# ShioMisaka/fce-yolo

Hardware: AMD Instinct MI355X
Metric: images/sec/GPU @ 640x640 bs=32, yolo11n-fce; fraction of fp16 MFMA roofline (higher is better)
Workload: dtype fp16; 1 GPU; yolo11n-fce detection inference (forward + decode + NMS) @ 640x640, 32 images/GPU; model=yolo11n-fce, global_batch=32, imgsz=640, parallelism=dp1, batches_in_flight=4, distinct_inputs=5, hw_queues=8, forward_launch=hipgraph

## Files before the change

fce-yolo_amd/_native.py:

```python

from __future__ import annotations

import ctypes as C
import os
from pathlib import Path

LIB_PATH = Path(__file__).resolve().parent / "lib" / "libfceyolo.so"

F16, F32, U8 = 0, 1, 2
NHWC, NCHW = 0, 1
ACT_NONE, ACT_SILU = 0, 1
EPI_STORE, EPI_WSTORE, EPI_ACCUM = 0, 1, 2
PLAN_NO_AUTOTUNE = 1


class FceError(RuntimeError):
    pass


class Tensor(C.Structure):
    _fields_ = [
        ("data", C.c_void_p),
        ("dtype", C.c_int),
        ("layout", C.c_int),
# ... 100 lines not shown
        ("w", C.c_void_p * 2),
        ("b", C.c_void_p * 2),
        ("epi1", C.c_int),
        ("fw", C.c_void_p),
        ("fn", C.c_int),
        ("fi", C.c_int),
    ]


class NmsOpts(C.Structure):
    _fields_ = [
        ("conf_thres", C.c_float),
        ("iou_thres", C.c_float),
        ("max_det", C.c_int),
        ("max_nms", C.c_int),
        ("max_wh", C.c_float),
        ("agnostic", C.c_int),
        ("multi_label", C.c_int),
        ("classes", C.c_void_p),
        ("nclasses", C.c_int),
    ]


_P = C.c_void_p
_I = C.c_int
_SZ = C.c_size_t
_PT = C.POINTER(Tensor)
_PCD = C.POINTER(ConvDesc)
_PCO = C.POINTER(CoordDesc)
_PC3 = C.POINTER(C3k2Desc)
_PDC = C.POINTER(DclsDesc)
_PST = C.POINTER(Stem2Desc)
_PBN = C.POINTER(BneckDesc)
_PPW = C.POINTER(Pw2Desc)

_SIGS = {
    "fce_last_error": (C.c_char_p, []),
    "fce_abi_version": (_I, []),
    "fce_device_count": (_I, []),
    "fce_conv_weight_bytes": (_SZ, [_PCD]),
    "fce_conv_pack_weights": (_I, [_PCD, _P, _P]),
    "fce_conv2d": (_I, [_PCD, _PT, _P, _P, _PT, _PT, _P]),
    "fce_conv_variants": (_I, [_PCD, _I, _P, _I]),
    "fce_letterbox": (_I, [_P, _I, _P, _I, _I, _I, _P]),
    "fce_scale_boxes": (_I, [_P, _P, _I, _I, _P, _P]),
    "fce_conv2d_variant": (_I, [_PCD, _PT, _P, _P, _PT, _PT, _I, _P]),
    "fce_conv2d_variant_dup": (_I, [_PCD, _PT, _P, _P, _PT, _PT, _I, _PT, _I, _P]),
    "fce_conv2d_detect": (_I, [_PCD, _PT, _P, _P, C.POINTER(DetectEpi), _P]),
    "fce_maxpool_chain": (_I, [_PT, _PT, _PT, _PT, _I, _P]),
    "fce_weighted_add": (_I, [_PT, _I, _P, _I, _I, _I, _PT, _P]),
    "fce_coord_workspace_bytes": (_SZ, [_PCO, _I, _I, _I]),
    "fce_c3k2_supported": (_I, [_PC3]),
    "fce_c3k2": (_I, [_PC3, _PT, _PT, _P]),
    "fce_net_add_c3k2": (_I, [_P, _PC3, _I, _I, _I, _I]),
    "fce_net_add_c3k2_alt": (_I, [_P, _PC3, _I, _I, _I, _I, _I, _I]),
    "fce_net_c3k2_form": (_I, [_P, _I]),
    "fce_net_set_c3k2_form": (_I, [_P, _I, _I]),
    "fce_net_op_skipped": (_I, [_P, _I]),
    "fce_detect_cls_supported": (_I, [_PDC]),
    "fce_detect_cls": (_I, [_PDC, _PT, C.POINTER(DetectEpi), _P]),
    "fce_net_add_detect_cls_alt": (_I, [_P, _PDC, _I, _I, _I, _I]),
    "fce_net_alt_form": (_I, [_P, _I]),
    "fce_stem_fused_supported": (_I, [_PST]),
    "fce_stem_fused": (_I, [_PST, _PT, _PT, _P]),
    "fce_net_add_stem_alt": (_I, [_P, _PST, _I, _I]),
    "fce_net_set_alt_form": (_I, [_P, _I, _I]),
    "fce_bneck_supported": (_I, [_PBN]),
    "fce_bneck_fused": (_I, [_PBN, _PT, _PT, _P]),
    "fce_net_add_bneck_alt": (_I, [_P, _PBN, _I, _I, _I, _I, _I, _I]),
    "fce_pw2_supported": (_I, [_PPW]),
    "fce_pw2": (_I, [_PPW, _PT, _PT, _PT, _I, _PT, _PT, _PT, _PT, _I, _P]),
    "fce_net_add_pw2_alt": (_I, [_P, _PPW, _I]),
    "fce_bicoordcrossatt": (_I, [_PCO, _PT, _PT, _P, _SZ, _P]),
    "fce_coordatt": (_I, [_PCO, _PT, _PT, _P, _SZ, _P]),
    "fce_coordcrossatt": (_I, [_PCO, _PT, _PT, _P, _SZ, _P]),
    "fce_psa_attention": (_I, [_PT, _I, _I, _I, _P, _P, _PT, _P]),
    "fce_detect_decode": (_I, [_PT, _PT, _I, _P, _I, _P, _P]),
    "fce_nms_workspace_bytes": (_SZ, [_I, _I, _I]),
    "fce_nms": (_I, [_P, _I, _I, _I, C.c_float, C.c_float, _I, _I, C.c_float, _P, _SZ, _P, _P, _P, _P]),
    "fce_nms_best": (_I, [_P, _P, _I, _I, _I, C.c_float, C.c_float, _I, _I, C.c_float, _P, _SZ, _P, _P, _P, _P]),
    "fce_nms_workspace_bytes_ex": (_SZ, [_I, _I, _I, C.POINTER(NmsOpts)]),
    "fce_nms_ex": (_I, [_P, _P, _I, _I, _I, C.POINTER(NmsOpts), _P, _SZ, _P, _P, _P, _P]),
    "fce_copy": (_I, [_PT, _PT, _P]),
    "fce_net_create": (_P, []),
    "fce_net_destroy": (None, [_P]),
    "fce_net_add_buffer": (_I, [_P, _I, _I, _I]),
    "fce_net_add_conv": (_I, [_P, _PCD, _I, _I, _I, _I, _I, _I, _P, _P]),
    "fce_net_add_conv_dup": (_I, [_P, _PCD, _I, _I, _I, _I, _I, _I, _P, _P, _I, _I, _I]),
    "fce_net_add_maxpool_chain": (_I, [_P, _I, _I, _I, _I]),
    "fce_net_add_weighted_add": (_I, [_P, _I, _I, _I, _I, _P, _I, _I, _I, _I, _I]),
    "fce_net_add_coord": (_I, [_P, _I, _PCO, _I, _I, _I, _I]),
    "fce_net_add_psa_attention": (_I, [_P, _I, _I, _I, _I, _P, _P, _I, _I]),
    "fce_net_add_detect": (_I, [_P, _I, _P, _P, _I]),
    "fce_net_add_conv_detect": (_I, [_P, _PCD, _I, _I, _I, _I, C.c_float, _I, _I, _P, _P]),
    "fce_net_plan": (_I, [_P, _I, _I, _I]),
    "fce_net_plan_ex": (_I, [_P, _I, _I, _I, _I]),
    "fce_net_arena_bytes": (_SZ, [_P]),
    "fce_net_num_anchors": (_I, [_P]),
    "fce_net_forward": (_I, [_P, _PT, _P, _I, _P]),
    "fce_net_forward_best": (_I, [_P, _PT, _P, _P, _I, _P]),
    "fce_net_fork_hint": (_I, [_P]),
    "fce_net_set_fork": (_I, [_P, _I]),
    "fce_net_wait_fork": (_I, [_P, _P]),
    "fce_net_profile": (_I, [_P, _PT, _P, _P, _P, _I, _P]),
    "fce_net_num_ops": (_I, [_P]),
    "fce_net_op_variant": (_I, [_P, _I]),
# ... 46 lines not shown
```

fce-yolo_amd/csrc/api.hip:

```cpp
#include "ops.h"

namespace fce {

static thread_local std::string g_err;
static thread_local LaunchProbe* g_probe = nullptr;
LaunchProbe*& probe_slot() { return g_probe; }
void set_error(const std::string& m) { g_err = m; }
int fail(int code, const std::string& m) {
  g_err = m;
  return code;
}
int check_nhwc(const fce_tensor* t, const char* name, int dtype) {
  if (!t) return fail(FCE_ERR_INVALID, std::string(name) + ": null tensor");
  if (t->layout != FCE_NHWC || t->dtype != dtype) return fail(FCE_ERR_INVALID, std::string(name) + ": wrong layout/dtype");
  return FCE_OK;
}

}

using namespace fce;

extern "C" {

const char* fce_last_error(void) { return g_err.c_str(); }
int fce_abi_version(void) { return FCE_ABI_VERSION; }
int fce_device_count(void) {
  int n = 0;
  if (hipGetDeviceCount(&n) != hipSuccess) {
    (void)hipGetLastError();
    return 0;
  }
  return n;
}

size_t fce_conv_weight_bytes(const fce_conv_desc* d) { return d ? conv_weight_bytes(*d) : 0; }
int fce_conv_pack_weights(const fce_conv_desc* d, const float* w, void* out) {
  FCE_CHECK(d && w && out, "fce_conv_pack_weights: null argument");
  FCE_GUARD(return conv_pack(*d, w, out);)
}
int fce_conv2d(const fce_conv_desc* d, const fce_tensor* x, const void* w, const float* bias, const fce_tensor* res,
               const fce_tensor* y, void* stream) {
  FCE_CHECK(d && x && w && bias && y, "fce_conv2d: null argument");
  FCE_GUARD(return conv2d(*d, *x, w, bias, res, *y, S(stream));)
}
int fce_conv_variants(const fce_conv_desc* d, int in_w, int* codes, int cap) {
  if (!d || !codes || cap <= 0) return 0;
  return conv_tile_candidates(*d, 0, in_w, codes, cap);
}
int fce_conv2d_variant(const fce_conv_desc* d, const fce_tensor* x, const void* w, const float* bias,
                       const fce_tensor* res, const fce_tensor* y, int variant, void* stream) {
  FCE_CHECK(d && x && w && bias && y, "fce_conv2d_variant: null argument");
  FCE_GUARD(return conv2d(*d, *x, w, bias, res, *y, S(stream), variant);)
}
int fce_conv2d_variant_dup(const fce_conv_desc* d, const fce_tensor* x, const void* w, const float* bias,
                           const fce_tensor* res, const fce_tensor* y, int variant, const fce_tensor* dup, int dup_lo,
                           void* stream) {
  FCE_CHECK(d && x && w && bias && y && dup, "fce_conv2d_variant_dup: null argument");
  FCE_CHECK(d->k == 1 && d->groups == 1 && d->epilogue == FCE_EPI_STORE && dup->dtype == FCE_F16 &&
                dup->layout == FCE_NHWC && dup_lo >= 0 && dup_lo % 8 == 0 && dup->c % 8 == 0 &&
                dup_lo + dup->c <= d->cout && dup->n == y->n && dup->h == y->h && dup->w == y->w,
            "fce_conv2d_variant_dup: the duplicate store needs a plain 1x1 conv and an aligned f16 view of y's size");
  FCE_GUARD(return conv2d(*d, *x, w, bias, res, *y, S(stream), variant, dup, dup_lo);)
}
int fce_c3k2_supported(const fce_c3k2_desc* d) { return d && c3k2_fused_ok(*d) ? 1 : 0; }
int fce_c3k2(const fce_c3k2_desc* d, const fce_tensor* x, const fce_tensor* y, void* stream) {
  FCE_CHECK(d && x && y, "fce_c3k2: null argument");
  FCE_GUARD(return c3k2_fused(*d, *x, *y, S(stream));)
}
int fce_detect_cls_supported(const fce_dcls_desc* d) { return d && detect_cls_fused_ok(*d) ? 1 : 0; }
int fce_detect_cls(const fce_dcls_desc* d, const fce_tensor* x, const fce_detect_epi* e, void* stream) {
  FCE_CHECK(d && x && e, "fce_detect_cls: null argument");
  FCE_GUARD(return detect_cls_fused(*d, *x, *e, S(stream));)
}
int fce_bneck_supported(const fce_bneck_desc* d) { return d && bneck_fused_ok(*d) ? 1 : 0; }
int fce_bneck_fused(const fce_bneck_desc* d, const fce_tensor* x, const fce_tensor* y, void* stream) {
  FCE_CHECK(d && x && y, "fce_bneck_fused: null argument");
  FCE_GUARD(return bneck_fused(*d, *x, *y, S(stream));)
}
int fce_pw2_supported(const fce_pw2_desc* d) { return d && pw2_fused_ok(*d) ? 1 : 0; }
int fce_pw2(const fce_pw2_desc* d, const fce_tensor* x1, const fce_tensor* r1, const fce_tensor* h, int h_store,
            const fce_tensor* x2, const fce_tensor* r2, const fce_tensor* y, const fce_tensor* dup, int dup_lo,
            void* stream) {
  FCE_CHECK(d && x1 && h && x2 && y, "fce_pw2: null argument");
  FCE_GUARD(return pw2_fused(*d, *x1, r1, *h, h_store, *x2, r2, *y, dup, dup_lo, S(stream));)
}
int fce_stem_fused_supported(const fce_stem2_desc* d) { return d && stem_fused_ok(*d) ? 1 : 0; }
int fce_stem_fused(const fce_stem2_desc* d, const fce_tensor* x, const fce_tensor* y, void* stream) {
  FCE_CHECK(d && x && y, "fce_stem_fused: null argument");
  FCE_GUARD(return stem_fused(*d, *x, *y, S(stream));)
}
int fce_conv2d_detect(const fce_conv_desc* d, const fce_tensor* x, const void* w, const float* bias,
                      const fce_detect_epi* e, void* stream) {
  FCE_CHECK(d && x && w && bias && e, "fce_conv2d_detect: null argument");
  FCE_GUARD(return conv2d_detect(*d, *x, w, bias, *e, S(stream));)
}
int fce_maxpool_chain(const fce_tensor* x, const fce_tensor* y1, const fce_tensor* y2, const fce_tensor* y3, int k,
                      void* stream) {
  FCE_CHECK(x && y1 && y2 && y3, "fce_maxpool_chain: null argument");
  FCE_GUARD(return maxpool_chain(*x, *y1, *y2, *y3, k, S(stream));)
}
int fce_weighted_add(const fce_tensor* x, int up, const float* fw, int fn, int fi, int accumulate, const fce_tensor* y,
                     void* stream) {
  FCE_CHECK(x && y, "fce_weighted_add: null argument");
  FCE_GUARD(return weighted_add(*x, up, fw, fn, fi, accumulate, *y, S(stream));)
}
size_t fce_coord_workspace_bytes(const fce_coord_desc* d, int n, int h, int w) {
  return d ? coord_ws_bytes(*d, n, h, w) : 0;
}
int fce_bicoordcrossatt(const fce_coord_desc* d, const fce_tensor* x, const fce_tensor* y, void* ws, size_t wsb,
                        void* stream) {
  FCE_CHECK(d && x && y, "fce_bicoordcrossatt: null argument");
  FCE_GUARD(return bicoordcrossatt(*d, *x, *y, ws, wsb, S(stream));)
}
int fce_coordatt(const fce_coord_desc* d, const fce_tensor* x, const fce_tensor* y, void* ws, size_t wsb,
                 void* stream) {
  FCE_CHECK(d && x && y, "fce_coordatt: null argument");
  FCE_GUARD(return coordatt(*d, *x, *y, ws, wsb, S(stream));)
}
int fce_coordcrossatt(const fce_coord_desc* d, const fce_tensor* x, const fce_tensor* y, void* ws, size_t wsb,
                      void* stream) {
// ... 51 lines not shown
```

fce-yolo_amd/csrc/fused.hip:

```cpp
#include <algorithm>

#include "mfma_stage.h"
#include "ops.h"

namespace fce {

static __device__ __attribute__((aligned(16))) _Float16 g_c3_zero[8];

template <int CIN, int C, int CM, int COUT, int TH, int TW, int NW>
struct C3G {
  static constexpr int R2W = TW + 4, R2 = (TH + 4) * R2W;
  static constexpr int R1W = TW + 2, R1 = (TH + 2) * R1W;
  static constexpr int NC = TH * TW;
  static constexpr int NF1 = (R2 + 15) / 16, NF2 = (R1 + 15) / 16, NF4 = (NC + 15) / 16;
  static constexpr int MF1 = (NF1 + NW - 1) / NW, MF2 = (NF2 + NW - 1) / NW, MF4 = (NF4 + NW - 1) / NW;
  static constexpr int CT1 = 2 * C / 16, CT2 = (CM + 15) / 16, CT3 = (C + 15) / 16, CT4 = (COUT + 15) / 16;
  static constexpr bool F2 = C % 32 == 0, F3 = CM % 32 == 0;
  static constexpr int NS1 = CIN / 32, NS2 = (9 * (C / 8) + 3) / 4, NS3 = (9 * (CM / 8) + 3) / 4,
                       NS4 = (3 * C / 8 + 3) / 4;
  static constexpr int sT = (2 * C / 8) | 1, sH = (CM / 8) | 1, sM = (C / 8) | 1;
  static constexpr int W1 = CT1 * NS1 * 64, W2 = CT2 * NS2 * 64, W3 = CT3 * NS3 * 64, W4 = CT4 * NS4 * 64;
  static constexpr int OW2 = W1, OW3 = W1 + W2, OW4 = W1 + W2 + W3, OB = W1 + W2 + W3 + W4;
  static constexpr int B2 = CT1 * 16, B3 = B2 + CT2 * 16, B4 = B3 + CT3 * 16, NB = B4 + CT4 * 16;
  static constexpr int OT = OB + NB / 4, OH = OT + R2 * sT, OM = OH + R1 * sH, TOTAL = OM + NC * sM;
  static constexpr size_t LDS = size_t(TOTAL) * 16;
  static_assert(CIN % 32 == 0 && C % 8 == 0 && CM % 8 == 0 && COUT % 8 == 0, "c3k2 fused: channel alignment");
};

struct C3k2Args {
  const _Float16* x;
  int xcs;
  _Float16* y;
  int ycs;
  int H, W, tiles_x, tiles_y, ntiles;
  const h8* w[4];
  int nalloc[4];
  const float* b[4];
  int diag;
};

__device__ __forceinline__ void c3_act(const float* bias, int ct, int grp, const f4& acc, float (&v)[4]) {
  const int co0 = ct * 16 + grp * 4;
#pragma unroll
  for (int j = 0; j < 4; ++j) v[j] = silu(acc[j] + bias[co0 + j]);
}

template <bool FAST, int CPT>
__device__ __forceinline__ void c3_kstep(int st, int grp, int& tap, int& cc, bool& ok) {
  if (FAST) {
    tap = st % 9;
    cc = (st / 9) * 4 + grp;
    ok = true;
  } else {
    const int k = st * 4 + grp;
    tap = k / CPT;
    cc = k - tap * CPT;
    ok = tap < 9;
  }
}

__device__ __forceinline__ void c3_tile(const C3k2Args& a, int TH, int TW, int t, int& n, int& y0, int& x0) {
  const int tx = t % a.tiles_x;
  t /= a.tiles_x;
  const int ty = t % a.tiles_y;
  n = t / a.tiles_y;
  y0 = ty * TH;
  x0 = tx * TW;
}

template <int CIN, int C, int CM, int COUT, int TH, int TW, int NW, bool YB>
__global__ __launch_bounds__(NW * 64, 2) void c3k2_fused_kernel(C3k2Args a) {
  using G = C3G<CIN, C, CM, COUT, TH, TW, NW>;
  extern __shared__ __attribute__((aligned(16))) h8 sm[];
  const int lane = threadIdx.x & 63, wave = threadIdx.x >> 6, col = lane & 15, grp = lane >> 4;
  const int NG = gridDim.x, bi = blockIdx.x;
  const int t_begin = int(int64_t(bi) * a.ntiles / NG), t_end = int(int64_t(bi + 1) * a.ntiles / NG);
  if (t_begin >= t_end) return;

  h8 xb[G::MF1][G::NS1];
  auto load_x = [&](int t) {
    int n, y0, x0;
    c3_tile(a, TH, TW, t, n, y0, x0);
    const _Float16* zl = g_c3_zero;
#pragma unroll
    for (int i = 0; i < G::MF1; ++i) {
      const int q = (wave + NW * i) * 16 + col;
      const int r = q / G::R2W, cq = q - r * G::R2W;
      const int iy = y0 - 2 + r, ix = x0 - 2 + cq;
      const bool in = q < G::R2 && iy >= 0 && iy < a.H && ix >= 0 && ix < a.W;
      const _Float16* src = a.x + (in ? nhwc_off(n, iy, ix, a.H, a.W, a.xcs) + grp * 8 : 0);
#pragma unroll
      for (int s = 0; s < G::NS1; ++s) xb[i][s] = *reinterpret_cast<const h8*>(in ? src + s * 32 : zl);
    }
  };
  load_x(t_begin);
  {
    const int wofs[4] = {0, G::OW2, G::OW3, G::OW4}, cts[4] = {G::CT1, G::CT2, G::CT3, G::CT4};
    const int nss[4] = {G::NS1, G::NS2, G::NS3, G::NS4}, couts[4] = {2 * C, CM, C, COUT};
    const int bofs[4] = {0, G::B2, G::B3, G::B4};
    float* bias = reinterpret_cast<float*>(sm + G::OB);
#pragma unroll
    for (int s = 0; s < 4; ++s) {
      stage_copy_frags(sm + wofs[s], a.w[s], cts[s], nss[s], a.nalloc[s], NW * 64);
      for (int e = int(threadIdx.x); e < cts[s] * 16; e += NW * 64) bias[bofs[s] + e] = e < couts[s] ? a.b[s][e] : 0.f;
    }
  }
  __syncthreads();

  const float* bias = reinterpret_cast<const float*>(sm + G::OB);
  _Float16* T = reinterpret_cast<_Float16*>(sm + G::OT);
  _Float16* Hh = reinterpret_cast<_Float16*>(sm + G::OH);
  _Float16* Mm = reinterpret_cast<_Float16*>(sm + G::OM);
  const h8* Tin = sm + G::OT;
  const h8* Hin = sm + G::OH;
  const h8* Min = sm + G::OM;
  uint64_t clk[6] = {0, 0, 0, 0, 0, 0}, tprev = a.diag ? __builtin_amdgcn_s_memtime() : 0;
  auto tick = [&](int k) {
    if (a.diag) {
      const uint64_t tn = __builtin_amdgcn_s_memtime();
      clk[k] += tn - tprev;
      tprev = tn;
    }
  };

  for (int t = t_begin; t < t_end; ++t) {
    int n, y0, x0;
    c3_tile(a, TH, TW, t, n, y0, x0);
    {
      auto bl = [&](int i, int st) -> h8 { return xb[i][st]; };
      auto epi = [&](int i, int ct, const f4& acc) {
        const int q = (wave + NW * i) * 16 + col;
        if (q >= G::R2) return;
        const int r = q / G::R2W, cq = q - r * G::R2W;
        const int iy = y0 - 2 + r, ix = x0 - 2 + cq;
        float v[4];
        c3_act(bias, ct, grp, acc, v);
        h4 o = h4_of(v);
        if (!(iy >= 0 && iy < a.H && ix >= 0 && ix < a.W)) o = h4{0, 0, 0, 0};
        *reinterpret_cast<h4*>(T + (q * G::sT) * 8 + ct * 16 + grp * 4) = o;
      };
      mfma_stage<G::MF1, G::CT1, G::NS1>(sm + lane, bl, epi);
    }
    tick(0);
    if (t + 1 < t_end) load_x(t + 1);
    tick(1);
    stage_barrier();
    {
      int pb[G::MF2];
#pragma unroll
      for (int i = 0; i < G::MF2; ++i) {
        const int q = min((wave + NW * i) * 16 + col, G::R1 - 1);
        const int r = q / G::R1W, cq = q - r * G::R1W;
        pb[i] = r * G::R2W + cq;
      }
      auto bl = [&](int i, int st) -> h8 {
        int tap, cc;
        bool ok;
        c3_kstep<G::F2, C / 8>(st, grp, tap, cc, ok);
        const int ky = tap / 3, kx = tap - ky * 3;
        return ok ? Tin[(pb[i] + ky * G::R2W + kx) * G::sT + C / 8 + cc] : h8{0, 0, 0, 0, 0, 0, 0, 0};
      };
      auto epi = [&](int i, int ct, const f4& acc) {
        const int q = (wave + NW * i) * 16 + col;
        if (q >= G::R1 || ct * 16 + grp * 4 >= CM) return;
        const int r = q / G::R1W, cq = q - r * G::R1W;
        const int iy = y0 - 1 + r, ix = x0 - 1 + cq;
        float v[4];
        c3_act(bias + G::B2, ct, grp, acc, v);
        h4 o = h4_of(v);
        if (!(iy >= 0 && iy < a.H && ix >= 0 && ix < a.W)) o = h4{0, 0, 0, 0};
        *reinterpret_cast<h4*>(Hh + (q * G::sH) * 8 + ct * 16 + grp * 4) = o;
      };
      mfma_stage<G::MF2, G::CT2, G::NS2>(sm + G::OW2 + lane, bl, epi);
    }
    tick(2);
    stage_barrier();
    {
      int pb[G::MF4];
#pragma unroll
      for (int i = 0; i < G::MF4; ++i) {
        const int q = min((wave + NW * i) * 16 + col, G::NC - 1);
        const int r = q / TW, cq = q - r * TW;
        pb[i] = r * G::R1W + cq;
      }
      auto bl = [&](int i, int st) -> h8 {
        int tap, cc;
        bool ok;
        c3_kstep<G::F3, CM / 8>(st, grp, tap, cc, ok);
        const int ky = tap / 3, kx = tap - ky * 3;
        return ok ? Hin[(pb[i] + ky * G::R1W + kx) * G::sH + cc] : h8{0, 0, 0, 0, 0, 0, 0, 0};
      };
      auto epi = [&](int i, int ct, const f4& acc) {
        const int q = (wave + NW * i) * 16 + col;
        const int co0 = ct * 16 + grp * 4;
        if (q >= G::NC || co0 >= C) return;
        const int r = q / TW, cq = q - r * TW;
        float v[4];
        c3_act(bias + G::B3, ct, grp, acc, v);
        const h4 rv = *reinterpret_cast<const h4*>(T + (((r + 2) * G::R2W + cq + 2) * G::sT) * 8 + C + co0);
#pragma unroll
        for (int j = 0; j < 4; ++j) v[j] = fpin(v[j] + (float)rv[j]);
        *reinterpret_cast<h4*>(Mm + (q * G::sM) * 8 + co0) = h4_of(v);
      };
      mfma_stage<G::MF4, G::CT3, G::NS3>(sm + G::OW3 + lane, bl, epi);
    }
    tick(3);
    stage_barrier();
    {
      int pt[G::MF4], pm[G::MF4];
#pragma unroll
      for (int i = 0; i < G::MF4; ++i) {
        const int q = min((wave + NW * i) * 16 + col, G::NC - 1);
        const int r = q / TW, cq = q - r * TW;
        pt[i] = ((r + 2) * G::R2W + cq + 2) * G::sT;
        pm[i] = q * G::sM - 2 * C / 8;
      }
      auto bl = [&](int i, int st) -> h8 {
        const int cc = st * 4 + grp;
        if (cc >= 3 * C / 8) return h8{0, 0, 0, 0, 0, 0, 0, 0};
        return cc < 2 * C / 8 ? Tin[pt[i] + cc] : Min[pm[i] + cc];
      };
      const uint32_t img = uint32_t(a.H) * uint32_t(a.W) * uint32_t(a.ycs);
      const __amdgpu_buffer_rsrc_t yr = out_rsrc(a.y + int64_t(n) * img, img * 2u);
      auto epi = [&](int i, int ct, const f4& acc) {
        const int q = (wave + NW * i) * 16 + col;
        const int r = q / TW, cq = q - r * TW;
        const int iy = y0 + r, ix = x0 + cq;
        const bool ok = q < G::NC && ct * 16 + grp * 4 < COUT && iy < a.H && ix < a.W;
        if (!YB && !ok) return;
        float v[4];
        c3_act(bias + G::B4, ct, grp, acc, v);
        const int off = (iy * a.W + ix) * a.ycs + ct * 16 + grp * 4;
        if constexpr (YB) store_h4_or_drop(yr, ok, uint32_t(off) * 2u, h4_of(v));
        else *reinterpret_cast<h4*>(a.y + int64_t(n) * img + off) = h4_of(v);
      };
      mfma_stage<G::MF4, G::CT4, G::NS4>(sm + G::OW4 + lane, bl, epi);
    }
    tick(4);
    stage_barrier();
    tick(5);
  }
  if (a.diag && blockIdx.x == 0 && threadIdx.x == 0) {
    const unsigned long long nt = (unsigned long long)(t_end - t_begin);
    printf("c3k2 fused diag: %llu tiles, clocks per tile: stage1 %llu, x-issue %llu, stage2 %llu, stage3 %llu, "
           "stage4 %llu, last barrier %llu\n", nt, (unsigned long long)clk[0] / nt, (unsigned long long)clk[1] / nt,
           (unsigned long long)clk[2] / nt, (unsigned long long)clk[3] / nt, (unsigned long long)clk[4] / nt,
           (unsigned long long)clk[5] / nt);
  }
}

struct C3Inst {
  int cin, c, cm, cout;
};
static constexpr C3Inst kC3Insts[] = {{32, 16, 8, 64}, {64, 32, 16, 128}, {32, 32, 16, 64}};

template <int CIN, int C, int CM, int COUT, int TH, int TW, int NW, bool YB>
static int c3_launch(const C3k2Args& a0, int H, int W, int N, hipStream_t s) {
  using G = C3G<CIN, C, CM, COUT, TH, TW, NW>;
  static_assert(G::LDS <= 160 * 1024, "c3k2 fused: LDS over 160 KiB");
  auto k = c3k2_fused_kernel<CIN, C, CM, COUT, TH, TW, NW, YB>;
  static const bool big = hipFuncSetAttribute(reinterpret_cast<const void*>(k),
                                              hipFuncAttributeMaxDynamicSharedMemorySize, 160 * 1024) == hipSuccess;
  if (!big && G::LDS > 64 * 1024) return fail(FCE_ERR_HIP, "c3k2 fused: cannot opt in to >64 KiB LDS");
  C3k2Args a = a0;
  a.tiles_x = (W + TW - 1) / TW;
  a.tiles_y = (H + TH - 1) / TH;
  const int64_t tiles = int64_t(a.tiles_x) * a.tiles_y * N;
  if (tiles == 0) return FCE_OK;
  FCE_CHECK(tiles < (int64_t(1) << 30), "c3k2 fused: grid too large");
  a.ntiles = int(tiles);
  static int cus = 0;
  if (!cus) {
    int dev = 0;
    if (hipGetDevice(&dev) != hipSuccess || hipDeviceGetAttribute(&cus, hipDeviceAttributeMultiprocessorCount, dev) != hipSuccess)
      cus = 256;
  }
  int occ = 0;
  if (hipOccupancyMaxActiveBlocksPerMultiprocessor(&occ, k, NW * 64, G::LDS) != hipSuccess || occ < 1) occ = 1;
  {
    static const int cap = [] {
      const char* e = getenv("FCE_C3K2_OCC");
      return e ? atoi(e) : 0;
    }();
    if (cap > 0) occ = std::min(occ, cap);
  }
  const int grid = int(std::min<int64_t>(a.ntiles, int64_t(cus) * occ));
  FCE_LAUNCH(k, dim3(unsigned(grid)), dim3(NW * 64), G::LDS, s, a);
  return launch_status("c3k2_fused_kernel");
}

template <int CIN, int C, int CM, int COUT>
static int c3_launch_cfg(const C3k2Args& a, int H, int W, int N, hipStream_t s) {
  const char* env = getenv("FCE_C3K2_TILE");
  bool wide = W >= 128;
  if (env && *env) {
    if (strcmp(env, "8,16,4") == 0) wide = true;
    else if (strcmp(env, "4,40,8") == 0) wide = false;
    else return fail(FCE_ERR_INVALID, "FCE_C3K2_TILE: only \"8,16,4\" or \"4,40,8\"");
  }
  const char* yst = getenv("FCE_C3K2_YSTORE");
  bool yb = COUT <= 64;
  if (yst && *yst) {
    if (strcmp(yst, "buf") == 0) yb = true;
    else if (strcmp(yst, "global") == 0) yb = false;
    else return fail(FCE_ERR_INVALID, "FCE_C3K2_YSTORE: only \"buf\" or \"global\"");
  }
  if (wide) return yb ? c3_launch<CIN, C, CM, COUT, 8, 16, 4, true>(a, H, W, N, s) : c3_launch<CIN, C, CM, COUT, 8, 16, 4, false>(a, H, W, N, s);
  return yb ? c3_launch<CIN, C, CM, COUT, 4, 40, 8, true>(a, H, W, N, s) : c3_launch<CIN, C, CM, COUT, 4, 40, 8, false>(a, H, W, N, s);
}

static int c3_inst(const fce_c3k2_desc& d) {
  for (int i = 0; i < int(sizeof(kC3Insts) / sizeof(kC3Insts[0])); ++i)
    if (kC3Insts[i].cin == d.cin && kC3Insts[i].c == d.c && kC3Insts[i].cm == d.c_mid && kC3Insts[i].cout == d.cout)
      return i;
  return -1;
}

bool c3k2_fused_ok(const fce_c3k2_desc& d) { return c3_inst(d) >= 0; }

int c3k2_fused(const fce_c3k2_desc& d, const fce_tensor& x, const fce_tensor& y, hipStream_t s) {
  const int inst = c3_inst(d);
  FCE_CHECK(inst >= 0, "c3k2 fused: unsupported channel configuration");
  FCE_CHECK(x.layout == FCE_NHWC && y.layout == FCE_NHWC && x.dtype == FCE_F16 && y.dtype == FCE_F16,
            "c3k2 fused: NHWC f16 views");
  FCE_CHECK(x.c == d.cin && y.c == d.cout && x.n == y.n && x.h == y.h && x.w == y.w, "c3k2 fused: shape mismatch");
  FCE_CHECK(x.cstride % 8 == 0 && x.coff % 8 == 0 && y.cstride % 4 == 0 && y.coff % 4 == 0,
            "c3k2 fused: aligned channel slices");
  for (int i = 0; i < 4; ++i) FCE_CHECK(d.w[i] && d.b[i], "c3k2 fused: null weights");
  C3k2Args a{};
  a.x = static_cast<const _Float16*>(x.data) + x.coff;
  a.xcs = x.cstride;
  a.y = static_cast<_Float16*>(y.data) + y.coff;
  a.ycs = y.cstride;
  a.H = x.h;
  a.W = x.w;
  const int cins[4] = {d.cin, d.c, d.c_mid, 3 * d.c}, ks[4] = {1, 3, 3, 1};
  for (int i = 0; i < 4; ++i) {
    a.w[i] = static_cast<const h8*>(d.w[i]);
    a.b[i] = d.b[i];
    a.nalloc[i] = stage_nalloc(cins[i], ks[i]);
  }
  {
    const char* de = getenv("FCE_C3K2_DIAG");
    a.diag = de && atoi(de) != 0;
  }
  switch (inst) {
    case 0: return c3_launch_cfg<32, 16, 8, 64>(a, x.h, x.w, x.n, s);
    case 1: return c3_launch_cfg<64, 32, 16, 128>(a, x.h, x.w, x.n, s);
    default: return c3_launch_cfg<32, 32, 16, 64>(a, x.h, x.w, x.n, s);
  }
}

}
```

fce-yolo_amd/csrc/ops.h:

```cpp
#pragma once
#include <exception>

#include "common.h"

namespace fce {

size_t conv_weight_bytes(const fce_conv_desc& d);
int conv_pack(const fce_conv_desc& d, const float* w, void* out);
int conv2d(const fce_conv_desc& d, const fce_tensor& x, const void* w, const float* bias, const fce_tensor* res,
           const fce_tensor& y, hipStream_t s, int tile = -1, const fce_tensor* dup = nullptr, int duplo = 0);
int conv2d_detect(const fce_conv_desc& d, const fce_tensor& x, const void* w, const float* bias,
                  const fce_detect_epi& e, hipStream_t s, int tile = -1);
int conv_tile_candidates(const fce_conv_desc& d, int det_box, int in_w, int* out, int cap);
int maxpool_chain(const fce_tensor& x, const fce_tensor& y1, const fce_tensor& y2, const fce_tensor& y3, int k,
                  hipStream_t s);
int weighted_add(const fce_tensor& x, int up, const float* fw, int fn, int fi, int accumulate, const fce_tensor& y,
                 hipStream_t s);
int copy(const fce_tensor& src, const fce_tensor& dst, hipStream_t s);
size_t coord_ws_bytes(const fce_coord_desc& d, int n, int h, int w);
int bicoordcrossatt(const fce_coord_desc& d, const fce_tensor& x, const fce_tensor& y, void* ws, size_t wsb,
                    hipStream_t s);
int coordatt(const fce_coord_desc& d, const fce_tensor& x, const fce_tensor& y, void* ws, size_t wsb, hipStream_t s);
int coordcrossatt(const fce_coord_desc& d, const fce_tensor& x, const fce_tensor& y, void* ws, size_t wsb,
                  hipStream_t s);
int psa_attention(const fce_tensor& qkv, int heads, int key_dim, int head_dim, const float* pe_w, const float* pe_b,
                  const fce_tensor& y, hipStream_t s);
int detect_decode(const fce_tensor* box, const fce_tensor* cls, int nl, const float* strides, int reg_max,
                  float* out, hipStream_t s);
size_t nms_ws_bytes(int n, int A, int max_nms);
size_t nms_ws_bytes_ex(int n, int nc, int A, int max_nms, int multi);
int nms(const float* pred, const unsigned long long* best, int n, int nc, int A, float conf, float iou, int max_det,
        int max_nms, float max_wh, void* ws, size_t ws_bytes, float* dets, int64_t* keep, int32_t* counts,
        hipStream_t s, int multi = 0, const int32_t* classes = nullptr, int nclasses = 0);
bool c3k2_fused_ok(const fce_c3k2_desc& d);
int c3k2_fused(const fce_c3k2_desc& d, const fce_tensor& x, const fce_tensor& y, hipStream_t s);
bool detect_cls_fused_ok(const fce_dcls_desc& d);
int detect_cls_fused(const fce_dcls_desc& d, const fce_tensor& x, const fce_detect_epi& e, hipStream_t s);
bool stem_fused_ok(const fce_stem2_desc& d);
bool stem_fused_fits(const fce_stem2_desc& d, int h, int w);
int stem_fused(const fce_stem2_desc& d, const fce_tensor& x, const fce_tensor& y, hipStream_t s);
bool bneck_fused_ok(const fce_bneck_desc& d);
bool bneck_fused_fits(const fce_bneck_desc& d, int h, int w);
int bneck_fused(const fce_bneck_desc& d, const fce_tensor& x, const fce_tensor& y, hipStream_t s);
bool pw2_fused_ok(const fce_pw2_desc& d);
int pw2_fused(const fce_pw2_desc& d, const fce_tensor& x1, const fce_tensor* r1, const fce_tensor& h, int h_store,
              const fce_tensor& x2, const fce_tensor* r2, const fce_tensor& y, const fce_tensor* dup, int dup_lo,
              hipStream_t s);
int letterbox(const fce_letterbox_img* imgs, int n, uint8_t* dst, int H, int W, int pad, hipStream_t s);
int scale_boxes(float* dets, const int32_t* counts, int n, int max_det, const fce_box_scale* sc, hipStream_t s);

}

#define FCE_GUARD(...)                                                          \
  try {                                                                         \
    __VA_ARGS__                                                                 \
  } catch (const std::exception& e) {                                           \
    return ::fce::fail(FCE_ERR_INVALID, std::string("exception: ") + e.what()); \
  } catch (...) {                                                               \
    return ::fce::fail(FCE_ERR_INVALID, "unknown exception");                   \
  }
```

include/fce_yolo.h:

```cpp
#ifndef FCE_YOLO_H
#define FCE_YOLO_H

#include <stddef.h>
#include <stdint.h>

#ifdef __cplusplus
extern "C" {
#endif

#define FCE_ABI_VERSION 7

#define FCE_OK 0
#define FCE_ERR_INVALID 1
#define FCE_ERR_HIP 2
#define FCE_ERR_UNSUPPORTED 3

#define FCE_F16 0
#define FCE_F32 1
#define FCE_U8 2
#define FCE_NHWC 0
#define FCE_NCHW 1
#define FCE_ACT_NONE 0
#define FCE_ACT_SILU 1
#define FCE_EPI_STORE 0
// ... 42 lines not shown
  unsigned long long* best;
} fce_detect_epi;
int fce_conv2d_detect(const fce_conv_desc* d, const fce_tensor* x, const void* w_packed, const float* bias,
                      const fce_detect_epi* e, void* stream);

typedef struct fce_letterbox_img {
  const uint8_t* src;
  int h0, w0, row_stride;
  int new_h, new_w;
  int top, left;
} fce_letterbox_img;
int fce_letterbox(const fce_letterbox_img* imgs, int n, uint8_t* dst, int H, int W, int pad_value, void* stream);
typedef struct fce_box_scale {
  float gain;
  int pad_x, pad_y, h0, w0;
} fce_box_scale;
int fce_scale_boxes(float* dets, const int32_t* counts, int n, int max_det, const fce_box_scale* params, void* stream);

int fce_maxpool_chain(const fce_tensor* x, const fce_tensor* y1, const fce_tensor* y2, const fce_tensor* y3, int k,
                      void* stream);
int fce_weighted_add(const fce_tensor* x, int up, const float* fusion_w, int fusion_n, int fusion_i, int accumulate,
                     const fce_tensor* y, void* stream);

typedef struct fce_coord_desc {
  int inp, oup, mid, heads;
  float scale;
  const float* w[8];
  const float* b[8];
  const void* id_w;
  const float* id_b;
} fce_coord_desc;

size_t fce_coord_workspace_bytes(const fce_coord_desc* d, int n, int h, int w);
int fce_bicoordcrossatt(const fce_coord_desc* d, const fce_tensor* x, const fce_tensor* y, void* ws, size_t ws_bytes,
                        void* stream);
int fce_coordatt(const fce_coord_desc* d, const fce_tensor* x, const fce_tensor* y, void* ws, size_t ws_bytes,
                 void* stream);
int fce_coordcrossatt(const fce_coord_desc* d, const fce_tensor* x, const fce_tensor* y, void* ws, size_t ws_bytes,
                      void* stream);

int fce_psa_attention(const fce_tensor* qkv, int heads, int key_dim, int head_dim, const float* pe_w,
                      const float* pe_b, const fce_tensor* y, void* stream);

int fce_detect_decode(const fce_tensor* box, const fce_tensor* cls, int nl, const float* strides, int reg_max,
                      float* out, void* stream);

typedef struct fce_c3k2_desc {
  int cin, c, c_mid, cout;
  const void* w[4];
  const float* b[4];
} fce_c3k2_desc;
int fce_c3k2_supported(const fce_c3k2_desc* d);
int fce_c3k2(const fce_c3k2_desc* d, const fce_tensor* x, const fce_tensor* y, void* stream);

typedef struct fce_dcls_desc {
  int c0, c3, nc;
  const void* w[5];
  const float* b[5];
} fce_dcls_desc;
int fce_detect_cls_supported(const fce_dcls_desc* d);
int fce_detect_cls(const fce_dcls_desc* d, const fce_tensor* x, const fce_detect_epi* e, void* stream);

typedef struct fce_stem2_desc {
  int c0, c1;
  const void* w[2];
  const float* b[2];
} fce_stem2_desc;
int fce_stem_fused_supported(const fce_stem2_desc* d);
int fce_stem_fused(const fce_stem2_desc* d, const fce_tensor* x, const fce_tensor* y, void* stream);

typedef struct fce_bneck_desc {
  int c, c_mid, n, shortcut;
  const void* w[4];
  const float* b[4];
} fce_bneck_desc;
int fce_bneck_supported(const fce_bneck_desc* d);
int fce_bneck_fused(const fce_bneck_desc* d, const fce_tensor* x, const fce_tensor* y, void* stream);

typedef struct fce_pw2_desc {
  int cin1, cout1, cin2, cout2;
  int act[2];
  const void* w[2];
  const float* b[2];
  int epi1;
  const float* fw;
  int fn, fi;
} fce_pw2_desc;
int fce_pw2_supported(const fce_pw2_desc* d);
int fce_pw2(const fce_pw2_desc* d, const fce_tensor* x1, const fce_tensor* r1, const fce_tensor* h, int h_store,
            const fce_tensor* x2, const fce_tensor* r2, const fce_tensor* y, const fce_tensor* dup, int dup_lo,
            void* stream);

size_t fce_nms_workspace_bytes(int n, int anchors, int max_nms);
int fce_nms(const float* pred, int n, int nc, int anchors, float conf_thres, float iou_thres, int max_det,
            int max_nms, float max_wh, void* ws, size_t ws_bytes, float* dets, int64_t* keep, int32_t* counts,
            void* stream);
int fce_nms_best(const float* pred, const unsigned long long* best, int n, int nc, int anchors, float conf_thres,
                 float iou_thres, int max_det, int max_nms, float max_wh, void* ws, size_t ws_bytes, float* dets,
                 int64_t* keep, int32_t* counts, void* stream);

typedef struct fce_nms_opts {
  float conf_thres, iou_thres;
  int max_det, max_nms;
  float max_wh;
  int agnostic, multi_label;
  const int32_t* classes;
// ... 66 lines not shown
```

Before: 39570 images/sec.

## Walk c3k2 fused tiles down columns and reuse halo rows via ring buffers

Reorders the fused C3k2 kernel's tile traversal so each block walks vertically through tiles (y fastest) when TH==4. Intermediate t and h rows stay in LDS ring buffers, so steady-state tiles only compute the new rows instead of recomputing the halo. This removes the redundant halo recomputation of stages 1 and 2, which is large for 4-row tiles. The cost is extra ring-index arithmetic, a second specialisation per stage, and more code paths. An env var can disable it, and a host helper exposes the walk order for testing.

```diff
diff --git a/fce-yolo_amd/_native.py b/fce-yolo_amd/_native.py
--- a/fce-yolo_amd/_native.py
+++ b/fce-yolo_amd/_native.py
@@ -176,6 +176,7 @@
     "fce_coord_workspace_bytes": (_SZ, [_PCO, _I, _I, _I]),
     "fce_c3k2_supported": (_I, [_PC3]),
     "fce_c3k2": (_I, [_PC3, _PT, _PT, _P]),
+    "fce_c3k2_walk_run": (_I, [_I, _I, _I, _I, _I, _I, _I, _P, _I, _P]),
     "fce_net_add_c3k2": (_I, [_P, _PC3, _I, _I, _I, _I]),
     "fce_net_add_c3k2_alt": (_I, [_P, _PC3, _I, _I, _I, _I, _I, _I]),
     "fce_net_c3k2_form": (_I, [_P, _I]),
diff --git a/fce-yolo_amd/csrc/api.hip b/fce-yolo_amd/csrc/api.hip
--- a/fce-yolo_amd/csrc/api.hip
+++ b/fce-yolo_amd/csrc/api.hip
@@ -66,6 +66,9 @@
 int fce_c3k2(const fce_c3k2_desc* d, const fce_tensor* x, const fce_tensor* y, void* stream) {
   FCE_CHECK(d && x && y, "fce_c3k2: null argument");
   FCE_GUARD(return c3k2_fused(*d, *x, *y, S(stream));)
+}
+int fce_c3k2_walk_run(int h, int w, int n, int th, int tw, int grid, int block, int* out, int cap, int* count) {
+  FCE_GUARD(return c3k2_walk_run(h, w, n, th, tw, grid, block, out, cap, count);)
 }
 int fce_detect_cls_supported(const fce_dcls_desc* d) { return d && detect_cls_fused_ok(*d) ? 1 : 0; }
 int fce_detect_cls(const fce_dcls_desc* d, const fce_tensor* x, const fce_detect_epi* e, void* stream) {
diff --git a/fce-yolo_amd/csrc/fused.hip b/fce-yolo_amd/csrc/fused.hip
--- a/fce-yolo_amd/csrc/fused.hip
+++ b/fce-yolo_amd/csrc/fused.hip
@@ -1,4 +1,5 @@
 #include <algorithm>
+#include <type_traits>
 
 #include "mfma_stage.h"
 #include "ops.h"
@@ -14,6 +15,11 @@
   static constexpr int NC = TH * TW;
   static constexpr int NF1 = (R2 + 15) / 16, NF2 = (R1 + 15) / 16, NF4 = (NC + 15) / 16;
   static constexpr int MF1 = (NF1 + NW - 1) / NW, MF2 = (NF2 + NW - 1) / NW, MF4 = (NF4 + NW - 1) / NW;
+  static constexpr int RH2 = TH + 4, RH1 = TH + 2;
+  static constexpr int S2 = TH * R2W, S1 = TH * R1W;
+  static constexpr int NF1S = (S2 + 15) / 16, NF2S = (S1 + 15) / 16;
+  static constexpr int MF1S = (NF1S + NW - 1) / NW, MF2S = (NF2S + NW - 1) / NW;
+  static_assert(TH >= 4, "c3k2 fused: the walk carries 4 rows of t, all from the previous tile");
   static constexpr int CT1 = 2 * C / 16, CT2 = (CM + 15) / 16, CT3 = (C + 15) / 16, CT4 = (COUT + 15) / 16;
   static constexpr bool F2 = C % 32 == 0, F3 = CM % 32 == 0;
   static constexpr int NS1 = CIN / 32, NS2 = (9 * (C / 8) + 3) / 4, NS3 = (9 * (CM / 8) + 3) / 4,
@@ -59,41 +65,65 @@
   }
 }
 
-__device__ __forceinline__ void c3_tile(const C3k2Args& a, int TH, int TW, int t, int& n, int& y0, int& x0) {
-  const int tx = t % a.tiles_x;
-  t /= a.tiles_x;
-  const int ty = t % a.tiles_y;
-  n = t / a.tiles_y;
-  y0 = ty * TH;
-  x0 = tx * TW;
-}
-
-template <int CIN, int C, int CM, int COUT, int TH, int TW, int NW, bool YB>
+__host__ __device__ inline void c3_run(int ntiles, int grid, int bi, int& t0, int& t1) {
+  t0 = int(int64_t(bi) * ntiles / grid);
+  t1 = int(int64_t(bi + 1) * ntiles / grid);
+}
+
+__host__ __device__ inline void c3_tile(bool walk, int tiles_x, int tiles_y, int t, int& n, int& ty, int& tx) {
+  if (walk) {
+    ty = t % tiles_y;
+    t /= tiles_y;
+    tx = t % tiles_x;
+    n = t / tiles_x;
+  } else {
+    tx = t % tiles_x;
+    t /= tiles_x;
+    ty = t % tiles_y;
+    n = t / tiles_y;
+  }
+}
+
+__host__ __device__ inline bool c3_first(int t, int t0, int tiles_y) { return t == t0 || t % tiles_y == 0; }
+
+template <bool RING, int RH>
+__device__ __forceinline__ int c3_ring(int v) {
+  return RING && v >= RH ? v - RH : v;
+}
+
+using c3_first_t = std::true_type;
+using c3_steady_t = std::false_type;
+
+template <int CIN, int C, int CM, int COUT, int TH, int TW, int NW, bool YB, bool WALK>
 __global__ __launch_bounds__(NW * 64, 2) void c3k2_fused_kernel(C3k2Args a) {
   using G = C3G<CIN, C, CM, COUT, TH, TW, NW>;
   extern __shared__ __attribute__((aligned(16))) h8 sm[];
   const int lane = threadIdx.x & 63, wave = threadIdx.x >> 6, col = lane & 15, grp = lane >> 4;
-  const int NG = gridDim.x, bi = blockIdx.x;
-  const int t_begin = int(int64_t(bi) * a.ntiles / NG), t_end = int(int64_t(bi + 1) * a.ntiles / NG);
+  int t_begin, t_end;
+  c3_run(a.ntiles, int(gridDim.x), int(blockIdx.x), t_begin, t_end);
   if (t_begin >= t_end) return;
+  auto is_first = [&](int t) { return !WALK || c3_first(t, t_begin, a.tiles_y); };
 
   h8 xb[G::MF1][G::NS1];
-  auto load_x = [&](int t) {
-    int n, y0, x0;
-    c3_tile(a, TH, TW, t, n, y0, x0);
+  auto load_x = [&](int t, auto kind) {
+    constexpr bool FIRST = decltype(kind)::value;
+    constexpr int MF = FIRST ? G::MF1 : G::MF1S, NP = FIRST ? G::R2 : G::S2, R0 = FIRST ? 0 : 4;
+    int n, ty, tx;
+    c3_tile(WALK, a.tiles_x, a.tiles_y, t, n, ty, tx);
+    const int y0 = ty * TH, x0 = tx * TW;
     const _Float16* zl = g_c3_zero;
 #pragma unroll
-    for (int i = 0; i < G::MF1; ++i) {
+    for (int i = 0; i < MF; ++i) {
       const int q = (wave + NW * i) * 16 + col;
       const int r = q / G::R2W, cq = q - r * G::R2W;
-      const int iy = y0 - 2 + r, ix = x0 - 2 + cq;
-      const bool in = q < G::R2 && iy >= 0 && iy < a.H && ix >= 0 && ix < a.W;
+      const int iy = y0 - 2 + R0 + r, ix = x0 - 2 + cq;
+      const bool in = q < NP && iy >= 0 && iy < a.H && ix >= 0 && ix < a.W;
       const _Float16* src = a.x + (in ? nhwc_off(n, iy, ix, a.H, a.W, a.xcs) + grp * 8 : 0);
 #pragma unroll
       for (int s = 0; s < G::NS1; ++s) xb[i][s] = *reinterpret_cast<const h8*>(in ? src + s * 32 : zl);
     }
   };
-  load_x(t_begin);
+  load_x(t_begin, c3_first_t{});
   {
     const int wofs[4] = {0, G::OW2, G::OW3, G::OW4}, cts[4] = {G::CT1, G::CT2, G::CT3, G::CT4};
     const int nss[4] = {G::NS1, G::NS2, G::NS3, G::NS4}, couts[4] = {2 * C, CM, C, COUT};
@@ -123,72 +153,95 @@
     }
   };
 
+  int rb2 = 0, rb1 = 0;
   for (int t = t_begin; t < t_end; ++t) {
-    int n, y0, x0;
-    c3_tile(a, TH, TW, t, n, y0, x0);
-    {
+    int n, ty, tx;
+    c3_tile(WALK, a.tiles_x, a.tiles_y, t, n, ty, tx);
+    const int y0 = ty * TH, x0 = tx * TW;
+    const bool first = is_first(t);
+    if (!WALK || first) rb2 = rb1 = 0;
+    int colf = col;
+    if (WALK) asm volatile("" : "+v"(colf));
+    auto stage1 = [&](auto kind) {
+      constexpr bool FIRST = decltype(kind)::value;
+      constexpr int MF = FIRST ? G::MF1 : G::MF1S, NP = FIRST ? G::R2 : G::S2, R0 = FIRST ? 0 : 4;
       auto bl = [&](int i, int st) -> h8 { return xb[i][st]; };
       auto epi = [&](int i, int ct, const f4& acc) {
-        const int q = (wave + NW * i) * 16 + col;
-        if (q >= G::R2) return;
+        const int q = (wave + NW * i) * 16 + (FIRST ? colf : col);
+        if (q >= NP) return;
         const int r = q / G::R2W, cq = q - r * G::R2W;
-        const int iy = y0 - 2 + r, ix = x0 - 2 + cq;
+        const int iy = y0 - 2 + R0 + r, ix = x0 - 2 + cq;
         float v[4];
         c3_act(bias, ct, grp, acc, v);
         h4 o = h4_of(v);
         if (!(iy >= 0 && iy < a.H && ix >= 0 && ix < a.W)) o = h4{0, 0, 0, 0};
-        *reinterpret_cast<h4*>(T + (q * G::sT) * 8 + ct * 16 + grp * 4) = o;
-      };
-      mfma_stage<G::MF1, G::CT1, G::NS1>(sm + lane, bl, epi);
-    }
+        const int p = FIRST ? q : c3_ring<true, G::RH2>(rb2 + R0 + r) * G::R2W + cq;
+        *reinterpret_cast<h4*>(T + (p * G::sT) * 8 + ct * 16 + grp * 4) = o;
+      };
+      mfma_stage<MF, G::CT1, G::NS1>(sm + lane, bl, epi);
+    };
+    if (first) stage1(c3_first_t{});
+    else stage1(c3_steady_t{});
     tick(0);
-    if (t + 1 < t_end) load_x(t + 1);
+    if (t + 1 < t_end) {
+      if (is_first(t + 1)) load_x(t + 1, c3_first_t{});
+      else load_x(t + 1, c3_steady_t{});
+    }
     tick(1);
     stage_barrier();
-    {
-      int pb[G::MF2];
-#pragma unroll
-      for (int i = 0; i < G::MF2; ++i) {
-        const int q = min((wave + NW * i) * 16 + col, G::R1 - 1);
-        const int r = q / G::R1W, cq = q - r * G::R1W;
-        pb[i] = r * G::R2W + cq;
+    auto stage2 = [&](auto kind) {
+      constexpr bool FIRST = decltype(kind)::value;
+      constexpr int MF = FIRST ? G::MF2 : G::MF2S, NP = FIRST ? G::R1 : G::S1, R0 = FIRST ? 0 : 2;
+      int pr[MF], pc[MF];
+#pragma unroll
+      for (int i = 0; i < MF; ++i) {
+        const int q = min((wave + NW * i) * 16 + (FIRST ? colf : col), NP - 1);
+        const int r = q / G::R1W;
+        pc[i] = q - r * G::R1W;
+        pr[i] = FIRST ? r : c3_ring<true, G::RH2>(rb2 + R0 + r);
       }
       auto bl = [&](int i, int st) -> h8 {
         int tap, cc;
         bool ok;
         c3_kstep<G::F2, C / 8>(st, grp, tap, cc, ok);
         const int ky = tap / 3, kx = tap - ky * 3;
-        return ok ? Tin[(pb[i] + ky * G::R2W + kx) * G::sT + C / 8 + cc] : h8{0, 0, 0, 0, 0, 0, 0, 0};
+        const int p = c3_ring<!FIRST, G::RH2>(pr[i] + ky) * G::R2W + pc[i] + kx;
+        return ok ? Tin[p * G::sT + C / 8 + cc] : h8{0, 0, 0, 0, 0, 0, 0, 0};
       };
       auto epi = [&](int i, int ct, const f4& acc) {
-        const int q = (wave + NW * i) * 16 + col;
-        if (q >= G::R1 || ct * 16 + grp * 4 >= CM) return;
+        const int q = (wave + NW * i) * 16 + (FIRST ? colf : col);
+        if (q >= NP || ct * 16 + grp * 4 >= CM) return;
         const int r = q / G::R1W, cq = q - r * G::R1W;
-        const int iy = y0 - 1 + r, ix = x0 - 1 + cq;
+        const int iy = y0 - 1 + R0 + r, ix = x0 - 1 + cq;
         float v[4];
         c3_act(bias + G::B2, ct, grp, acc, v);
         h4 o = h4_of(v);
         if (!(iy >= 0 && iy < a.H && ix >= 0 && ix < a.W)) o = h4{0, 0, 0, 0};
-        *reinterpret_cast<h4*>(Hh + (q * G::sH) * 8 + ct * 16 + grp * 4) = o;
-      };
-      mfma_stage<G::MF2, G::CT2, G::NS2>(sm + G::OW2 + lane, bl, epi);
-    }
+        const int p = FIRST ? q : c3_ring<true, G::RH1>(rb1 + R0 + r) * G::R1W + cq;
+        *reinterpret_cast<h4*>(Hh + (p * G::sH) * 8 + ct * 16 + grp * 4) = o;
+      };
+      mfma_stage<MF, G::CT2, G::NS2>(sm + G::OW2 + lane, bl, epi);
+    };
+    if (first) stage2(c3_first_t{});
+    else stage2(c3_steady_t{});
     tick(2);
     stage_barrier();
     {
-      int pb[G::MF4];
+      int pr[G::MF4], pc[G::MF4];
 #pragma unroll
       for (int i = 0; i < G::MF4; ++i) {
         const int q = min((wave + NW * i) * 16 + col, G::NC - 1);
-        const int r = q / TW, cq = q - r * TW;
-        pb[i] = r * G::R1W + cq;
+        const int r = q / TW;
+        pc[i] = q - r * TW;
+        pr[i] = c3_ring<WALK, G::RH1>(rb1 + r);
       }
       auto bl = [&](int i, int st) -> h8 {
         int tap, cc;
         bool ok;
         c3_kstep<G::F3, CM / 8>(st, grp, tap, cc, ok);
         const int ky = tap / 3, kx = tap - ky * 3;
-        return ok ? Hin[(pb[i] + ky * G::R1W + kx) * G::sH + cc] : h8{0, 0, 0, 0, 0, 0, 0, 0};
+        const int p = c3_ring<WALK, G::RH1>(pr[i] + ky) * G::R1W + pc[i] + kx;
+        return ok ? Hin[p * G::sH + cc] : h8{0, 0, 0, 0, 0, 0, 0, 0};
       };
       auto epi = [&](int i, int ct, const f4& acc) {
         const int q = (wave + NW * i) * 16 + col;
@@ -197,7 +250,8 @@
         const int r = q / TW, cq = q - r * TW;
         float v[4];
         c3_act(bias + G::B3, ct, grp, acc, v);
-        const h4 rv = *reinterpret_cast<const h4*>(T + (((r + 2) * G::R2W + cq + 2) * G::sT) * 8 + C + co0);
+        const int pt = c3_ring<WALK, G::RH2>(rb2 + r + 2) * G::R2W + cq + 2;
+        const h4 rv = *reinterpret_cast<const h4*>(T + (pt * G::sT) * 8 + C + co0);
 #pragma unroll
         for (int j = 0; j < 4; ++j) v[j] = fpin(v[j] + (float)rv[j]);
         *reinterpret_cast<h4*>(Mm + (q * G::sM) * 8 + co0) = h4_of(v);
@@ -212,7 +266,7 @@
       for (int i = 0; i < G::MF4; ++i) {
         const int q = min((wave + NW * i) * 16 + col, G::NC - 1);
         const int r = q / TW, cq = q - r * TW;
-        pt[i] = ((r + 2) * G::R2W + cq + 2) * G::sT;
+        pt[i] = (c3_ring<WALK, G::RH2>(rb2 + r + 2) * G::R2W + cq + 2) * G::sT;
         pm[i] = q * G::sM - 2 * C / 8;
       }
       auto bl = [&](int i, int st) -> h8 {
@@ -239,6 +293,10 @@
     tick(4);
     stage_barrier();
     tick(5);
+    if (WALK) {
+      rb2 = c3_ring<true, G::RH2>(rb2 + TH);
+      rb1 = c3_ring<true, G::RH1>(rb1 + TH);
+    }
   }
   if (a.diag && blockIdx.x == 0 && threadIdx.x == 0) {
     const unsigned long long nt = (unsigned long long)(t_end - t_begin);
@@ -254,11 +312,19 @@
 };
 static constexpr C3Inst kC3Insts[] = {{32, 16, 8, 64}, {64, 32, 16, 128}, {32, 32, 16, 64}};
 
-template <int CIN, int C, int CM, int COUT, int TH, int TW, int NW, bool YB>
+static bool c3_walk_enabled() {
+  static const bool on = [] {
+    const char* e = getenv("FCE_C3K2_WALK");
+    return !(e && *e && atoi(e) == 0);
+  }();
+  return on;
+}
+
+template <int CIN, int C, int CM, int COUT, int TH, int TW, int NW, bool YB, bool WALK>
 static int c3_launch(const C3k2Args& a0, int H, int W, int N, hipStream_t s) {
   using G = C3G<CIN, C, CM, COUT, TH, TW, NW>;
   static_assert(G::LDS <= 160 * 1024, "c3k2 fused: LDS over 160 KiB");
-  auto k = c3k2_fused_kernel<CIN, C, CM, COUT, TH, TW, NW, YB>;
+  auto k = c3k2_fused_kernel<CIN, C, CM, COUT, TH, TW, NW, YB, WALK>;
   static const bool big = hipFuncSetAttribute(reinterpret_cast<const void*>(k),
                                               hipFuncAttributeMaxDynamicSharedMemorySize, 160 * 1024) == hipSuccess;
   if (!big && G::LDS > 64 * 1024) return fail(FCE_ERR_HIP, "c3k2 fused: cannot opt in to >64 KiB LDS");
@@ -284,9 +350,26 @@
     }();
     if (cap > 0) occ = std::min(occ, cap);
   }
-  const int grid = int(std::min<int64_t>(a.ntiles, int64_t(cus) * occ));
+  int grid = int(std::min<int64_t>(a.ntiles, int64_t(cus) * occ));
+  {
+    const char* e = getenv("FCE_C3K2_GRID");
+    const int g = e ? atoi(e) : 0;
+    if (g > 0) grid = std::min(g, 1 << 16);
+  }
   FCE_LAUNCH(k, dim3(unsigned(grid)), dim3(NW * 64), G::LDS, s, a);
   return launch_status("c3k2_fused_kernel");
+}
+
+template <int CIN, int C, int CM, int COUT, int TH, int TW, int NW>
+static int c3_launch_tile(const C3k2Args& a, int H, int W, int N, hipStream_t s, bool yb) {
+  constexpr bool kWalk = TH == 4;
+  if constexpr (kWalk) {
+    if (c3_walk_enabled() && H > TH)
+      return yb ? c3_launch<CIN, C, CM, COUT, TH, TW, NW, true, true>(a, H, W, N, s)
+                : c3_launch<CIN, C, CM, COUT, TH, TW, NW, false, true>(a, H, W, N, s);
+  }
+  return yb ? c3_launch<CIN, C, CM, COUT, TH, TW, NW, true, false>(a, H, W, N, s)
+            : c3_launch<CIN, C, CM, COUT, TH, TW, NW, false, false>(a, H, W, N, s);
 }
 
 template <int CIN, int C, int CM, int COUT>
@@ -305,8 +388,25 @@
     else if (strcmp(yst, "global") == 0) yb = false;
     else return fail(FCE_ERR_INVALID, "FCE_C3K2_YSTORE: only \"buf\" or \"global\"");
   }
-  if (wide) return yb ? c3_launch<CIN, C, CM, COUT, 8, 16, 4, true>(a, H, W, N, s) : c3_launch<CIN, C, CM, COUT, 8, 16, 4, false>(a, H, W, N, s);
-  return yb ? c3_launch<CIN, C, CM, COUT, 4, 40, 8, true>(a, H, W, N, s) : c3_launch<CIN, C, CM, COUT, 4, 40, 8, false>(a, H, W, N, s);
+  if (wide) return c3_launch_tile<CIN, C, CM, COUT, 8, 16, 4>(a, H, W, N, s, yb);
+  return c3_launch_tile<CIN, C, CM, COUT, 4, 40, 8>(a, H, W, N, s, yb);
+}
+
+int c3k2_walk_run(int H, int W, int N, int th, int tw, int grid, int block, int* out, int cap, int* count) {
+  FCE_CHECK(H > 0 && W > 0 && N > 0 && th > 0 && tw > 0 && grid > 0 && block >= 0 && block < grid && cap >= 0 &&
+                (out || cap == 0) && count, "c3k2 walk run: bad argument");
+  const int tiles_x = (W + tw - 1) / tw, tiles_y = (H + th - 1) / th;
+  const int64_t tiles = int64_t(tiles_x) * tiles_y * N;
+  FCE_CHECK(tiles < (int64_t(1) << 30), "c3k2 walk run: grid too large");
+  int t0, t1;
+  c3_run(int(tiles), grid, block, t0, t1);
+  for (int t = t0; t < t1 && t - t0 < cap; ++t) {
+    int* o = out + 4 * (t - t0);
+    c3_tile(true, tiles_x, tiles_y, t, o[0], o[1], o[2]);
+    o[3] = c3_first(t, t0, tiles_y) ? 1 : 0;
+  }
+  *count = t1 - t0;
+  return FCE_OK;
 }
 
 static int c3_inst(const fce_c3k2_desc& d) {
diff --git a/fce-yolo_amd/csrc/ops.h b/fce-yolo_amd/csrc/ops.h
--- a/fce-yolo_amd/csrc/ops.h
+++ b/fce-yolo_amd/csrc/ops.h
@@ -34,6 +34,7 @@
         hipStream_t s, int multi = 0, const int32_t* classes = nullptr, int nclasses = 0);
 bool c3k2_fused_ok(const fce_c3k2_desc& d);
 int c3k2_fused(const fce_c3k2_desc& d, const fce_tensor& x, const fce_tensor& y, hipStream_t s);
+int c3k2_walk_run(int H, int W, int N, int th, int tw, int grid, int block, int* out, int cap, int* count);
 bool detect_cls_fused_ok(const fce_dcls_desc& d);
 int detect_cls_fused(const fce_dcls_desc& d, const fce_tensor& x, const fce_detect_epi& e, hipStream_t s);
 bool stem_fused_ok(const fce_stem2_desc& d);
diff --git a/include/fce_yolo.h b/include/fce_yolo.h
--- a/include/fce_yolo.h
+++ b/include/fce_yolo.h
@@ -118,6 +118,7 @@
 } fce_c3k2_desc;
 int fce_c3k2_supported(const fce_c3k2_desc* d);
 int fce_c3k2(const fce_c3k2_desc* d, const fce_tensor* x, const fce_tensor* y, void* stream);
+int fce_c3k2_walk_run(int h, int w, int n, int th, int tw, int grid, int block, int* out, int cap, int* count);
 
 typedef struct fce_dcls_desc {
   int c0, c3, nc;
```

Result: no change. 39820 images/sec, median of 6 (+0.6%).
